# hamza1030/stereo_matching_cuda

Measured on AMD Instinct MI355X. Metric: disparity MPix/s (stereo pair -> L+R disparity + occlusion-filled map), higher is better.
Workload: dtype f32; 1 GPU; kitti 1242x375 D=192 seeded synthetic pair (seed 20150101); width=1242, height=375, disparities=192, slices_in_flight=192, walker_launches_per_call=1

## Files before the change

stereo_matching_cuda_amd/csrc/smx_agg.hip:

```cpp
#include <string.h>

#include "smx_agg.h"
#include "smx_agg_v4.h"
#include "smx_agg_v5.h"
#include "smx_launch.h"
#include "smx_wta.h"

namespace smx {

constexpr int RING_TH_COLOR_MAX = 59745, RING_TH_GRAD_MAX = 59872;

static bool ring_applies(const smx_params* p, bool use_cost) {
    return v4_supported(p) && (use_cost || (p->th_color <= RING_TH_COLOR_MAX && p->th_grad <= RING_TH_GRAD_MAX));
}

static bool v5_applies(const smx_params* p, int w, int h, int nviews, bool use_cost) {
    return v5_fix_bytes(w, h, nviews) < 0x80000000ull &&
           (use_cost ? v5_supported_cost(p) && (size_t)w * h >= 4 : v5_supported(p));
}

int agg_path_for(const smx_params* p, int w, int h, int nviews, bool use_cost, int forced, const char** why) {
    *why = nullptr;
    if (forced == 1) return 1;
    if (!ring_applies(p, use_cost)) {
// ... 69 lines not shown
static_assert(WS_SLACK >= 255 + FIT_RESERVE, "a workspace sized for n slices holds n slices");
size_t agg_workspace_bytes(int w, int h, int nslices) {
    const AggLayout L = agg_layout(w, h, v4::RMAX, 1, true, true, true, nslices);
    return L.ctrl + agg_ctrl_bytes(L.K_flags, 2 * (size_t)nslices) + WS_COMB_COPY_SLACK + WS_SLACK;
}

int agg_plan(const smx_params* p, int w, int h, int nviews, bool use_cost, bool own_q, const AggOpts& opt, size_t ws_bytes,
             size_t lost, int total, AggLayout* L) {
    const bool comb = opt.walker != 4 && v5_applies(p, w, h, nviews, use_cost);
    const bool fallback = comb && use_cost;
    const char* why = nullptr;
    if (!agg_path_for(p, w, h, nviews, use_cost, opt.walker == 5 ? 5 : 3, &why)) return fail(SMX_E_ARG, "aggregate_fused: %s", why);
    if ((size_t)h * ((size_t)w + 2 * v4::PADX) * 8 >= 0x80000000ull)
        return fail(SMX_E_ARG, "aggregate_fused: an image plane of %d x %d exceeds 2 GiB", w, h);
    const size_t avail = ws_bytes > lost ? ws_bytes - lost : 0;
    *L = agg_layout(w, h, p->radius, nviews, comb, fallback, own_q, 0);
    if (L->fg[0] > avail) return fail(SMX_E_WS, "aggregate_fused: workspace too small");
    const size_t per_sv = L->q_slice + L->hand_sv * 4 + (size_t)L->K_flags * sizeof(unsigned);
    const size_t rest = avail > L->chunk_begin ? avail - L->chunk_begin : 0;
    const size_t fit = rest > FIT_RESERVE ? (rest - FIT_RESERVE) / (per_sv * nviews) : 0;
    if (L->chunk_begin > avail || (fit < 1 && total > 0))
        return fail(SMX_E_WS, "aggregate_fused: workspace %zu B too small (need >= %zu B per view)", ws_bytes,
                    agg_workspace_bytes(w, h, 1));
    int chunk = fit > (size_t)total ? total : (int)fit;
    if (opt.max_chunk > 0 && chunk > opt.max_chunk) chunk = opt.max_chunk;
    if (chunk < 1) chunk = 1;
    *L = agg_layout(w, h, p->radius, nviews, comb, fallback, own_q, chunk);
    if (L->end > avail) return fail(SMX_E_WS, "aggregate_fused: workspace carve overflow");
    return SMX_OK;
}

int agg_read_status(const void* d_ws, unsigned* out, int nwords) {
    const char* base = (const char*)align_up((size_t)d_ws, 256);
    SMX_HIP(hipMemcpy(out, base, sizeof(unsigned) * (size_t)nwords, hipMemcpyDeviceToHost));
    return SMX_OK;
}

static v5::Args comb_args(const v4::Args& a, const AggLayout& L, char* base, bool use_cost, bool fast) {
    v5::Args b;
    memset(&b, 0, sizeof(b));
    b.fix = base + L.fg[0];
    b.fix_bytes = L.fix_end - L.fg[0];
    for (int v = 0; v < 2; ++v) {
        const int vv = v < L.nviews ? v : 0;
        b.o_fg[v] = (unsigned)(L.fg[v] - L.fg[0]);
        b.o_g1p[v] = (unsigned)(L.g1p[vv] - L.fg[0]);
        b.o_i2p[v] = (unsigned)(L.i2p[vv] - L.fg[0]);
        b.q[v] = a.v[vv].q;
        b.d0[v] = a.v[vv].d0;
        b.cost[v] = a.v[vv].cost;
    }
    b.w = a.w; b.h = a.h; b.K = L.K; b.NI = L.NI;
    b.P = v5::period(a.h, L.K);
    b.nslices = a.nslices; b.nsv = a.nsv; b.nitems = a.nitems;
    b.hand = (float*)a.hand; b.flags = a.flags; b.ticket = a.ticket; b.status = a.status;
    b.src_cost = use_cost ? 1 : 0;
    b.cost_plane = L.plane;
    b.bad = a.status + 1;
    b.cc = a.cc;
    const _Float16 hc = (_Float16)a.cc.th_color, hg = (_Float16)a.cc.th_grad;
    unsigned short uc, ug;
    memcpy(&uc, &hc, 2); memcpy(&ug, &hg, 2);
    b.th2 = (unsigned)uc | ((unsigned)ug << 16);
    b.fast = fast ? 1 : 0;
    constexpr double PRIO_MAX_Q_BYTES = 6e9;
    const double q_bytes = (double)a.nsv * (double)L.qplane * 4.0;
    b.prio = q_bytes < PRIO_MAX_Q_BYTES ? 1 : 0;
    b.qperm = L.own_q ? 1 : 0;
    b.q_plane = L.qplane;
    return b;
}

static int guidance(const AggLayout& L, char* base, const AggCall& c, v4::Guidance* out) {
    const int nviews = L.nviews, w = c.w, h = c.h;
    const smx_params* const p = c.p;
    hipStream_t st = c.st;
    v4::Guidance& g = *out;
    memset(&g, 0, sizeof(g));
    g.I[0] = c.guide[0];
    g.I[1] = nviews == 2 ? c.guide[1] : c.other[0];
    for (int i = 0; i < 2; ++i) g.FG[i] = (aggdev::fg_t*)(base + L.fg[i]);
    for (int v = 0; v < nviews; ++v) {
        g.S0[v] = (float*)(base + L.scratch[v][0]); g.S1[v] = (float*)(base + L.scratch[v][1]);
        g.G[v] = (aggdev::f2*)(base + L.guid[v]);
        g.mean_u8[v] = c.mean_u8[v];
    }
    g.zero[0] = (unsigned*)(base + L.status); g.nzero[0] = 64;
    g.zero[1] = (unsigned*)(base + L.ctrl); g.nzero[1] = (unsigned)(L.ctrl_bytes / 4);
    int rc = v4_guidance_launch(g, nviews, w, h, p->radius, p->eps, !L.comb, st);
    if (rc || !L.comb) return rc;
    aggdev::f2* g1p[2] = {nullptr, nullptr};
    unsigned* i2p[2] = {nullptr, nullptr};
    for (int v = 0; v < nviews; ++v) { g1p[v] = (aggdev::f2*)(base + L.g1p[v]); i2p[v] = (unsigned*)(base + L.i2p[v]); }
    return v5_perm_launch(nviews, g.S0, g.S1, g.G, g.mean_u8, g.FG, g1p, i2p, w, h, p->eps, st);
}

static int aggregate_fused(const AggCall& c, const AggOpts& opt, AggInfo* info) {
    const smx_params* const p = c.p;
    const int nviews = c.nviews, w = c.w, h = c.h, s_begin = c.s_begin, s_end = c.s_end;
    hipStream_t st = c.st;
    const bool use_cost = c.cost[0] != nullptr;
    const bool own_q = !c.agg[0];
    float* const* const d_nbr = c.nbr[0] ? c.nbr : nullptr;
    float* const* const d_uq = c.uq[0] ? c.uq : nullptr;
    char* const base = (char*)align_up((size_t)c.ws, 256);
    AggLayout L;
    int rc = agg_plan(p, w, h, nviews, use_cost, own_q, opt, c.ws_bytes, (size_t)(base - (char*)c.ws), s_end - s_begin, &L);
    if (rc) return rc;
    info->walker_used = L.comb ? 5 : 4;
    info->chunk = L.chunk;
    if (opt.keys_fresh && s_end <= s_begin) {
        for (int v = 0; v < nviews; ++v)
            if ((rc = launch_init_keys(c.keys[v], (int64_t)w * h, st))) return rc;
    }
    unsigned* const status = (unsigned*)(base + L.status);
    char* const ctrl = base + L.ctrl;
    v4::Guidance g;
    if ((rc = guidance(L, base, c, &g))) return rc;
    int nl = 3;
    stage_mark(ST_GUIDANCE, st);

    v4::Args a0;
    memset(&a0, 0, sizeof(a0));
    a0.w = w; a0.h = h; a0.R = p->radius; a0.K = L.K; a0.NI = L.NI;
    a0.cc = make_cost_const(p);
    for (int v = 0; v < nviews; ++v) {
        a0.v[v].FG1 = g.FG[v]; a0.v[v].FG2 = g.FG[v ^ 1];
        a0.v[v].guid = g.G[v];
    }
    a0.hand = (aggdev::f2*)(base + L.hand);
    a0.ticket = (unsigned*)ctrl; a0.status = status;
    a0.flags = (unsigned*)(ctrl + AGG_CTRL_BYTES);
    const unsigned* const fell_back = L.fallback ? status + 1 : nullptr;
    for (int s0 = s_begin; s0 < s_end; s0 += L.chunk) {
        const int cnt = (s_end - s0) < L.chunk ? (s_end - s0) : L.chunk;
        v4::Args a = a0;
        const float* q[2] = {nullptr, nullptr};
        for (int v = 0; v < nviews; ++v) {
            a.v[v].q = own_q ? (float*)(base + L.q[v]) : c.agg[v] + (size_t)(s0 - s_begin) * L.plane;
            a.v[v].d0 = c.dmin[v] + s0;
            a.v[v].cost = use_cost ? c.cost[v] + (size_t)(s0 - s_begin) * L.plane : nullptr;
            q[v] = a.v[v].q;
        }
        a.nslices = cnt; a.nsv = cnt * nviews;
        a.nitems = a.nsv * L.K;
        const size_t ctrl_bytes = agg_ctrl_bytes(L.K_flags, a.nsv);
        if (s0 != s_begin) SMX_HIP(hipMemsetAsync(ctrl, 0, ctrl_bytes, st));
        if (L.comb) {
            rc = v5_launch(comb_args(a, L, base, use_cost, opt.fast), st);
            if (!rc && L.fallback) {
                SMX_HIP(hipMemsetAsync(ctrl, 0, ctrl_bytes, st));
                v4::Args a4 = a;
                a4.K = L.K4; a4.NI = L.NI4;
                a4.nitems = a4.nsv * L.K4;
                a4.gate = fell_back;
                rc = v4_walk_launch(a4, true, opt.fast, st);
                nl += 2;
            }
        } else rc = v4_walk_launch(a, use_cost, opt.fast, st);
        if (rc) return rc;
        ++info->walker_launches;
        stage_mark(ST_WALK, st);
        const bool fresh = opt.keys_fresh && s0 == s_begin;
        const bool comb_q = L.comb && own_q;
        rc = wta_launch(comb_q ? WTA_COMB : WTA_NATURAL, nviews, q, c.keys, d_nbr, d_uq, w, h, L.qplane, cnt, s0,
                        comb_q ? fell_back : nullptr, 0, fresh, st);
        if (!rc && comb_q && L.fallback) {
// ... 112 lines not shown
```

stereo_matching_cuda_amd/csrc/smx_agg_dev.h:

```cpp
#pragma once
#include "smx_common.h"

namespace smx {
namespace aggdev {

typedef _Float16 fg_t __attribute__((ext_vector_type(2)));
typedef float f2 __attribute__((ext_vector_type(2)));
typedef float f4 __attribute__((ext_vector_type(4)));
typedef unsigned u4 __attribute__((ext_vector_type(4)));
typedef unsigned u2 __attribute__((ext_vector_type(2)));

constexpr int PADX = 4;

constexpr int RCP_N = 19 * 19 + 1;
struct RcpTable {
    float v[RCP_N];
    constexpr RcpTable() : v() {
        v[0] = 0.0f;
        for (int i = 1; i < RCP_N; ++i) v[i] = 1.0f / (float)i;
    }
};
static __constant__ RcpTable kRcp = RcpTable();

__device__ __forceinline__ float div_small_int(float x, float d, float r) {
    float q = x * r;
    float e = __builtin_fmaf(-q, d, x);
    return __builtin_fmaf(e, r, q);
}
__device__ __forceinline__ f2 div_small_int2(f2 x, float d, float r) {
    const f2 d2 = {d, d}, r2 = {r, r};
    f2 q = x * r2;
    f2 e = __builtin_elementwise_fma(-q, d2, x);
    return __builtin_elementwise_fma(e, r2, q);
}
__device__ __forceinline__ bool div_needs_exact(float x) {
    const float ax = fabsf(x);
    return !(ax >= 0x1p-100f && ax < __builtin_inff());
}

__device__ __forceinline__ f2 guid_point(const float* __restrict__ S0, const float* __restrict__ S1, int x, int y, int w, int h,
                                         int R, double eps) {
    const int ymin = max(-1, y - R - 1), ymax = min(h - 1, y + R);
    const int xmin = max(-1, x - R - 1), xmax = min(w - 1, x + R);
    const bool hx = xmin >= 0, hy = ymin >= 0;
    const size_t i11 = (size_t)ymax * w + xmax, i10 = (size_t)ymax * w + (hx ? xmin : 0);
    const size_t i01 = (size_t)(hy ? ymin : 0) * w + xmax, i00 = (size_t)(hy ? ymin : 0) * w + (hx ? xmin : 0);
    const float area = (float)((xmax - xmin) * (ymax - ymin));
    auto box = [&](const float* __restrict__ S) {
        float val = S[i11];
        if (hx) val -= S[i10];
        if (hy) val -= S[i01];
        if (hx && hy) val += S[i00];
        return 1.0f * val / area;
    };
    const float m = box(S0), sq = box(S1);
    const float m2 = m * m;
    const float var = sq - m2;
    return (f2){m, (float)(1.0f / ((double)var + eps))};
}
__device__ __forceinline__ uint8_t mean_to_u8(float m) {
    const int ci = (int)m;
    return (ci > 255) ? 255 : (uint8_t)ci;
}

__device__ __forceinline__ f2 cost_pair(fg_t q1, fg_t q2, const CostConst& cc) {
    const f2 v1 = {(float)q1.x, (float)q1.y}, v2 = {(float)q2.x, (float)q2.y};
    const f2 d = v1 - v2;
    const f2 m = {__builtin_fminf(__builtin_fabsf(d.x), cc.th_color), __builtin_fminf(__builtin_fabsf(d.y), cc.th_grad)};
    const f2 xz = (f2){cc.oma, cc.alpha} * m;
    f2 r;
    r.x = xz.x + xz.y;
    r.y = v1.x * r.x;
    return r;
}

typedef __amdgpu_buffer_rsrc_t rsrc_t;
constexpr int AUX_SC1 = 16;
constexpr int AUX_NT = 2;
__device__ __forceinline__ rsrc_t mk_rsrc(const void* p, size_t bytes) {
    return __builtin_amdgcn_make_buffer_rsrc(const_cast<void*>(p), 0,
                                             (int)(bytes > 0xFFFFFFFFull ? 0xFFFFFFFFull : bytes),
                                             0x00020000);
}
__device__ __forceinline__ f4 ld16_sc1(rsrc_t r, unsigned byteoff) {
    return __builtin_bit_cast(f4, __builtin_amdgcn_raw_buffer_load_b128(r, (int)byteoff, 0, AUX_SC1));
}
__device__ __forceinline__ void st16_sc1(rsrc_t r, unsigned byteoff, f4 v) {
    __builtin_amdgcn_raw_buffer_store_b128(__builtin_bit_cast(u4, v), r, (int)byteoff, 0, AUX_SC1);
}
__device__ __forceinline__ unsigned ldu(rsrc_t r, unsigned voff, int soff) {
    return __builtin_amdgcn_raw_buffer_load_b32(r, (int)voff, soff, 0);
}
typedef __attribute__((address_space(1))) unsigned gu32;
__device__ __forceinline__ unsigned flag_load(unsigned* p) {
    return __hip_atomic_load((gu32*)p, __ATOMIC_RELAXED, __HIP_MEMORY_SCOPE_AGENT);
}
__device__ __forceinline__ void flag_store(unsigned* p, unsigned v) {
    __hip_atomic_store((gu32*)p, v, __ATOMIC_RELAXED, __HIP_MEMORY_SCOPE_AGENT);
}
__device__ __forceinline__ void drain_vmem() { asm volatile("s_waitcnt vmcnt(0)" ::: "memory"); }
__device__ __forceinline__ void wg_barrier() {
    asm volatile("s_waitcnt lgkmcnt(0)\n\ts_barrier" ::: "memory");
}

constexpr unsigned FLAG_DONE = 0x7fffffffu;
constexpr unsigned OOB = 0x80000000u;

__device__ __forceinline__ int opaque(int x) { asm volatile("" : "+v"(x)); return x; }
typedef __attribute__((address_space(3))) const char lds_cc;
__device__ __forceinline__ unsigned lds_off(const void* p) { return (unsigned)(size_t)(lds_cc*)p; }

}
}
```

stereo_matching_cuda_amd/csrc/smx_agg_v4.hip:

```cpp
#include <stdlib.h>
#include <string.h>

#include <type_traits>

#include "smx_agg_v4.h"

namespace smx {
namespace v4 {
using namespace aggdev;

constexpr int TWMAX = OW + HWMAX;
constexpr int NCOLP = 84;
constexpr int OFF1 = 88;
constexpr int ROWF = OFF1 + NCOLP;
static_assert(NCOLP >= TWMAX && NCOLP % 4 == 0 && OFF1 % 4 == 0 && OFF1 >= NCOLP, "planar ring row");
constexpr int NT = 512;
constexpr int NWAVE = NT / 64;
constexpr int RPW = BH / NWAVE;
constexpr int RR = BH + 2 * RMAX + 2;
static_assert(RR % 4 == 0 && RR % RPW == 0 && BH % RPW == 0 && RPW % 2 == 0,
              "groups of four (column scan) and of RPW (box, cost) consecutive ring rows never wrap");

enum Src { SRC_IMG = 0, SRC_COST = 1 };

// ... 65 lines not shown
                g = 1.0f * (c2 - c1) / 2;
            }
            fg_t v;
            v.x = (_Float16)f;
            v.y = (_Float16)g;
            FGo[(size_t)(y0 + r) * wp + xp] = v;
        }
    }
    if (view >= ga.nviews) return;
    __syncthreads();
    if (tid < 2 * rows) {
        float* row = gr_lds + tid * wpad;
        float acc = -0.0f;
        f4 c[16], n[16];
        auto rd = [&](f4 (&t)[16], int x0) {
#pragma unroll
            for (int k = 0; k < 16; ++k) t[k] = *(const f4*)(row + x0 + 4 * k);
        };
        auto scan_wr = [&](f4 (&t)[16], int x0) {
#pragma unroll
            for (int k = 0; k < 16; ++k) {
                acc = t[k].x + acc; t[k].x = acc;
                acc = t[k].y + acc; t[k].y = acc;
                acc = t[k].z + acc; t[k].z = acc;
                acc = t[k].w + acc; t[k].w = acc;
            }
#pragma unroll
            for (int k = 0; k < 16; ++k) *(f4*)(row + x0 + 4 * k) = t[k];
        };
        rd(c, 0);
        for (int x0 = 0; x0 < wr; x0 += 128) {
            rd(n, x0 + 64);
            scan_wr(c, x0);
            rd(c, min(x0 + 128, wr - 64));
            scan_wr(n, x0 + 64);
        }
    }
    __syncthreads();
    for (int r = 0; r < rows; ++r) {
        if (y0 + r >= h) break;
        float* d0 = S0 + (size_t)(y0 + r) * w;
        float* d1 = S1 + (size_t)(y0 + r) * w;
        for (int x = tid; x < w; x += GR_NT) {
            d0[x] = P0[r * wpad + x];
            d1[x] = P1[r * wpad + x];
        }
    }
}

constexpr int GC_NW = 16, GC_SEG = 32;
__global__ __launch_bounds__(64 * GC_NW) void k_v4_guid_cols(GuidArgs ga, int w, int h) {
    __shared__ float s_acc[64];
    __shared__ int s_turn;
    const int lane = threadIdx.x & 63, wv = threadIdx.x >> 6;
    const int x = blockIdx.x * 64 + lane;
    const bool on = x < w;
    float* __restrict__ p = ga.S[blockIdx.z][blockIdx.y] + min(x, w - 1);
    if (threadIdx.x == 0) s_turn = 0;
    __syncthreads();
    const int nseg = (h + GC_SEG - 1) / GC_SEG;
    float v[GC_SEG];
    for (int seg = wv; seg < nseg; seg += GC_NW) {
        const int y0 = seg * GC_SEG;
#pragma unroll
        for (int t = 0; t < GC_SEG; ++t) v[t] = p[(size_t)min(y0 + t, h - 1) * w];
        while (__hip_atomic_load(&s_turn, __ATOMIC_ACQUIRE, __HIP_MEMORY_SCOPE_WORKGROUP) != seg) __builtin_amdgcn_s_sleep(1);
        float acc = seg == 0 ? -0.0f : s_acc[lane];
#pragma unroll
        for (int t = 0; t < GC_SEG; ++t) { acc = v[t] + acc; v[t] = acc; }
        s_acc[lane] = acc;
        __builtin_amdgcn_fence(__ATOMIC_RELEASE, "workgroup");
        if (lane == 0) __hip_atomic_store(&s_turn, seg + 1, __ATOMIC_RELEASE, __HIP_MEMORY_SCOPE_WORKGROUP);
        if (on) {
#pragma unroll
            for (int t = 0; t < GC_SEG; ++t)
                if (y0 + t < h) p[(size_t)(y0 + t) * w] = v[t];
        }
    }
}

__global__ void k_v4_guid_finish(GuidArgs ga, int w, int h, int R, double eps) {
    const int x = blockIdx.x * blockDim.x + threadIdx.x, y = blockIdx.y, view = blockIdx.z;
    if (x >= w) return;
    const f2 g = guid_point(ga.S[view][0], ga.S[view][1], x, y, w, h, R, eps);
    const size_t id = (size_t)y * w + x;
    ga.G[view][id] = g;
    if (ga.mean_u8[view]) ga.mean_u8[view][id] = mean_to_u8(g.x);
}

constexpr int REC_U = REC_F2 / 2;
static_assert(REC_U <= NT && HP % 2 == 0 && BH % 2 == 0, "one 16-byte hand-off unit per thread");

constexpr int NQ = (TWMAX + 3) / 4;
constexpr int QW0 = 2;
constexpr int QTH = NT - 64 * QW0;
constexpr int NQR = BH / 16;
static_assert(NQ * 4 <= NCOLP && NQ <= 4 * (NWAVE - QW0), "one wave-instruction covers 16 rows x 4 quads");

#define LDS_RD64(dst, addr, imm) asm volatile("ds_read_b64 %0, %1 offset:%2" : "=v"(dst) : "v"(addr), "i"(imm))
#define LDS_RD2(dst, addr, o0, o1) \
    asm volatile("ds_read2_b32 %0, %1 offset0:%2 offset1:%3" : "=v"(dst) : "v"(addr), "i"(o0), "i"(o1))

template <int SRC, int RT, bool FAST>
__global__ __launch_bounds__(NT, 2 * WG_PER_CU) void k_v4_walk(Args A) {
    __shared__ __attribute__((aligned(16))) float ring1[RR * ROWF];
    __shared__ __attribute__((aligned(16))) float ring2[RR * ROWF];
    __shared__ __attribute__((aligned(16))) f2 cout[2][BH];
    __shared__ __attribute__((aligned(16))) f2 cin_fast[FAST ? 2 : 1][FAST ? BH : 1];
    __shared__ float rcp_s[HWMAX * HWMAX + 1];
    __shared__ int s_item, s_next;
    __shared__ unsigned s_seen;

    const int tid = threadIdx.x, lane = tid & 63;
    const int wave = __builtin_amdgcn_readfirstlane(tid >> 6);
    const int w = A.w, h = A.h, K = A.K, NI = A.NI, nsv = A.nsv;
    const int R = RT >= 0 ? RT : A.R;
    const int HW = 2 * R + 1, TW = OW + HW;
    const CostConst cc = A.cc;
    const f2 ident = {-0.0f, -0.0f};
    if (tid <= HWMAX * HWMAX) rcp_s[tid] = kRcp.v[tid];

    const int qt = tid - 64 * QW0;
    constexpr int NHALO_U = BH * HP / 2;
    static_assert(NHALO_U + BH <= QTH, "one hand-off unit per thread of waves QW0..");
    const bool hu_halo = qt >= 0 && qt < NHALO_U;
    const bool hu_carry = qt >= NHALO_U && qt < NHALO_U + BH;
    auto hu_rc = [&](int& r, int& c) {
        const int u = max(opaque(qt), 0);
        r = u / (HP / 2);
        c = (u - r * (HP / 2)) * 2;
    };
    auto hu_off = [&]() {
        const int u = opaque(qt);
        return u < NHALO_U ? (unsigned)(2 * BH * 8 + u * 16) : (unsigned)((u - NHALO_U) * 16);
    };
    auto srow_of = [&]() { return opaque(lane) & 15; };
    auto scomp_of = [&]() { return (opaque(lane) >> 4) & 1; };
    auto sstage_of = [&]() { return opaque(lane) >> 5; };
    constexpr int NRSW = 1;
    const bool q_on = wave >= QW0 && 4 * (wave - QW0) + (lane >> 4) < NQ;
    auto quad_rc = [&](int e, int& r, int& c) {
        const int l = opaque(lane);
        r = 16 * e + (l & 15);
        c = (4 * (wave - QW0) + (l >> 4)) * 4;
    };

    if (A.gate && flag_load(const_cast<unsigned*>(A.gate)) == 0u) return;
    if (tid == 0) s_item = (int)__hip_atomic_fetch_add((gu32*)A.ticket, 1u, __ATOMIC_RELAXED, __HIP_MEMORY_SCOPE_AGENT);
    for (;;) {
        wg_barrier();
        const int item = s_item;
        if (item >= A.nitems) break;
        const int k = item / nsv;
        const int sv = item - k * nsv;
        const int view = sv / A.nslices;
        const int slice = sv - view * A.nslices;
        const View& V = A.v[view];
        const int xs = k * OW;
        const int cs1 = xs - R - 1;
        const int cs2 = xs - HW;
        const bool pred = k > 0, succ = k + 1 < K;
        const int d = V.d0 + slice;
        unsigned* const myflag = A.flags + (size_t)sv * K + k;
        const size_t recs = (size_t)NI * REC_F2;
        const rsrc_t r_in = mk_rsrc(A.hand + ((size_t)((k - 1) & 1) * nsv + sv) * recs, recs * 8);
        const rsrc_t r_out = mk_rsrc(A.hand + ((size_t)(k & 1) * nsv + sv) * recs, recs * 8);

// ... 655 lines not shown
```

stereo_matching_cuda_amd/csrc/smx_agg_v5.hip:

```cpp
#include <stdlib.h>
#include <string.h>

#include <type_traits>

#include "smx_agg_dev.h"
#include "smx_agg_v5.h"
#include "smx_v5_diag.h"

namespace smx {
namespace v5 {
using namespace aggdev;

constexpr int SWU = HW * L;
constexpr int SW = (SWU + 3) / 4 * 4;
static_assert(OWS == HW * (L - 1) && SWU == OWS + HW && CPW * L <= 64 && CPW * NS1 >= HW, "strip geometry");
constexpr int RD = 20;
static_assert(RD % BH == 0 && RD >= HW + 1, "ring");
static_assert(L == 9, "the shipped form: seven combs of nine lanes per comb wave");
constexpr int NX = 2;
constexpr int NWAVE = 2 * NS1 + NX, NT = 64 * NWAVE;
constexpr int WPE = 4;
constexpr int NT1 = 3, NT2 = 2;
enum Role { ROLE_S1 = 0, ROLE_S2 = 1, ROLE_SCAN = 2, ROLE_COST = 3 };
constexpr int P1 = (SW + 63) / 64 * 64;
// ... 748 lines not shown
                        if (nxt < A.nitems) {
                            const int kn = nxt / nsv, svn = nxt - kn * nsv;
                            if (kn > 0) pn = flag_load(A.flags + (size_t)svn * K + kn - 1);
                        }
                        s_peekn = pn;
                    }
                }
                if (A.prio) __builtin_amdgcn_s_setprio(PRIO_COST);
                if (own && slf + 2 < NI) eval_band_p(slf + 2, G1[2]);
                __builtin_amdgcn_s_setprio(0);
            } else if constexpr (ROLE == ROLE_S1) {
                if (own) slot_s1(PARc, slf);
            } else {
                const int sl = sl2;
                if (own && sl >= 1 && sl <= q_last) {
                    slot_s2(PARc, sl);
                } else if (lane == 0) {
                    __hip_atomic_fetch_add(&s_x1, 1u, __ATOMIC_RELAXED, __HIP_MEMORY_SCOPE_WORKGROUP);
                }
            }
            have_pref = f_pred && (seen == FLAG_DONE || seen >= (unsigned)(slf + 3));
            if (f_pred && !have_pref && slf + 2 < NI) {
                if (tid == 0) spin_pred((unsigned)(slf + 3));
                wg_barrier();
                seen = s_seen;
                if constexpr (ROLE == ROLE_S1) {
                    const int hq = hu_idx();
                    const f4 late = ld16_sc1(r_hand, (unsigned)(o_in + min(slf + 2, NI - 1) * REC_U * 16) + (hq >= 0 && hq < REC_U ? (unsigned)hq * 16u : 0u));
                    cin1 = GC[1]; tile2 = G2[0];
                    hand_in(slf >= 0, late);
                }
            } else if constexpr (ROLE == ROLE_S1) {
                V5_MARK("s1handin begin");
                if (own && pred && slf + 2 < NI) { cin1 = GC[1]; tile2 = G2[0]; hand_in(slf >= 0, hreg); }
                V5_MARK("s1handin end");
            }
            if constexpr (ROLE == ROLE_S1) {
                g1_load(slf >= 0 ? 5 * slf + 6 : slf + 2, PARc);
                if (own && slf == 0 && succ) drain_vmem();
            }
            V5_STAMP(5);
            if (ending && slf == 1) return true;
            { float* const t = G1[0]; G1[0] = G1[1]; G1[1] = G1[2]; G1[2] = t; }
            { float* const t = G2[0]; G2[0] = G2[1]; G2[1] = t; }
            { float (*const t)[2] = GC[0]; GC[0] = GC[1]; GC[1] = t; }
            ++g;
            ++sl2;
            return false;
        };
        for (;;) {
            bool done = false;
            for (slf = -2; slf < 2 && !done; slf += 2) {
                done = iter(std::integral_constant<int, 0>{});
                if (!done) { ++slf; done = iter(std::integral_constant<int, 1>{}); --slf; }
            }
            if (done) break;
            for (slf = 2; slf <= P - 3; slf += 2) {
                (void)iter(std::integral_constant<int, 0>{});
                ++slf;
                (void)iter(std::integral_constant<int, 1>{});
                --slf;
            }
            ++nf;
        }
        if constexpr (ROLE == ROLE_COST) { if (own) cost_verdict(); }
        };
        if (wave < NS1) item_body(std::integral_constant<int, ROLE_S1>{});
        else if (wave < 2 * NS1) item_body(std::integral_constant<int, ROLE_S2>{});
        else if (wave == 2 * NS1) item_body(std::integral_constant<int, ROLE_SCAN>{});
        else item_body(std::integral_constant<int, ROLE_COST>{});
    }
}

struct PermArgs {
    const float* S0[2];
    const float* S1[2];
    f2* G[2];
    uint8_t* mean_u8[2];
    double eps;
    const fg_t* FG[2];
    f2* g1p[2];
    unsigned* i2p[2];
};
__global__ __launch_bounds__(CLP) void k_v5_perm(PermArgs pa, int w, int h, int K, int NI) {
    const int cl = threadIdx.x, cw = cl >> 6, ln = cl & 63;
    const int rho = ln / L < CPW ? CPW * cw + ln / L : HW, il = ln % L;
    const int kb = blockIdx.x / (BH / 2), j = blockIdx.x - kb * (BH / 2);
    const int k = kb / NI, ib = kb - k * NI, v = blockIdx.y;
    const int x1 = OWS * k - R - 1 + HW * il + rho;
    const int xq = x1 - R;
    const bool on1 = rho < HW && x1 >= 0 && x1 < w, on2 = rho < HW && xq >= 0 && xq < w;
    {
        const int ya = min(max(BH * ib - R + 2 * j, 0), h - 1), yb = min(max(BH * ib - R + 2 * j + 1, 0), h - 1);
        f4 g = {0.0f, 0.0f, 0.0f, 0.0f};
        if (on1) {
            const f2 a = guid_point(pa.S0[v], pa.S1[v], x1, ya, w, h, R, pa.eps);
            const f2 b = yb == ya ? a : guid_point(pa.S0[v], pa.S1[v], x1, yb, w, h, R, pa.eps);
            g = (f4){a.x, a.y, b.x, b.y};
            pa.G[v][(size_t)ya * w + x1] = a;
            pa.G[v][(size_t)yb * w + x1] = b;
            if (pa.mean_u8[v]) {
                pa.mean_u8[v][(size_t)ya * w + x1] = mean_to_u8(a.x);
                pa.mean_u8[v][(size_t)yb * w + x1] = mean_to_u8(b.x);
            }
        }
        ((f4*)pa.g1p[v])[((size_t)k * (5 * NI) + 5 * ib + j) * CLP + cl] = g;
    }
    {
        const int yp = min(max((BH * (ib - 1) - 2 * R) / 2 + j, 0), (h - 1) / 2), y = 2 * yp;
        fg_t p2 = {(_Float16)0.0f, (_Float16)0.0f};
        if (on2) {
            p2.x = pa.FG[v][(size_t)y * (w + 2 * PADX) + PADX + xq].x;
            if (y + 1 < h) p2.y = pa.FG[v][(size_t)(y + 1) * (w + 2 * PADX) + PADX + xq].x;
        }
        const unsigned pr = __builtin_bit_cast(unsigned, p2);
        unsigned* const i2a = pa.i2p[v];
        unsigned* const i2b = pa.i2p[v] + (size_t)K * NI * CLP * 4;
        const size_t e = ((size_t)k * NI + ib) * CLP + cl;
        if (j < 4) i2a[4 * e + j] = pr; else i2b[e] = pr;
    }
}

}

int v5_perm_launch(int nviews, const float* const* S0, const float* const* S1, aggdev::f2* const* G, uint8_t* const* mean_u8,
                   const aggdev::fg_t* const* FG, aggdev::f2* const* g1p, unsigned* const* i2p, int w, int h, double eps,
                   hipStream_t st) {
    v5::PermArgs pa;
    memset(&pa, 0, sizeof(pa));
    for (int v = 0; v < nviews; ++v) {
        pa.S0[v] = S0[v]; pa.S1[v] = S1[v]; pa.G[v] = G[v]; pa.mean_u8[v] = mean_u8[v];
        pa.FG[v] = FG[v]; pa.g1p[v] = g1p[v]; pa.i2p[v] = i2p[v];
    }
    pa.eps = eps;
    const int K = v5::strips(w), NI = v5::bands(h);
    hipLaunchKernelGGL(v5::k_v5_perm, dim3((unsigned)(K * NI * (v5::BH / 2)), (unsigned)nviews), dim3(v5::CLP), 0, st, pa, w, h, K, NI);
    SMX_HIP(hipGetLastError());
    return SMX_OK;
}

void v5_slots(int h, int K, int* bands, int* q_last, int* period) { *bands = v5::bands(h); *q_last = (h + 37) / 10; *period = v5::period(h, K); }

bool v5_supported(const smx_params* p) {
    if (p->radius != v5::R) return false;
    if (!(p->eps >= 1.0) || !(p->eps < 1e30)) return false;
    const CostConst c = make_cost_const(p);
    if (!(c.alpha >= 0.0f && c.alpha <= 1.0f && c.th_color >= 0.0f && c.th_color < 1e6f && c.th_grad >= 0.0f && c.th_grad < 1e6f))
        return false;
    const float m1 = c.th_color < 1.0f ? c.th_color : 1.0f, m2 = c.th_grad < 0.5f ? c.th_grad : 0.5f;
    const float t1 = c.oma * m1, t2 = c.alpha * m2;
    auto ok = [](float t) { return t == 0.0f || t >= 0x1p-60f; };
    if (!(ok(t1) && ok(t2))) return false;
    if (!((float)(_Float16)c.th_color == c.th_color && (float)(_Float16)c.th_grad == c.th_grad && c.th_color <= 59744.0f &&
          c.th_grad <= 59872.0f))
        return false;
    return true;
}

bool v5_supported_cost(const smx_params* p) { return p->radius == v5::R && p->eps >= 1.0 && p->eps < 1e30; }

int v5_launch(const v5::Args& a, hipStream_t st) {
    int dev = 0, ncu = 256;
    SMX_HIP(hipGetDevice(&dev));
    SMX_HIP(hipDeviceGetAttribute(&ncu, hipDeviceAttributeMultiprocessorCount, dev));
    const int slots = v5::WG_PER_CU * ncu;
    const int grid = a.nitems < slots ? a.nitems : slots;
    if (a.fast && a.qperm) hipLaunchKernelGGL((v5::k_v5_walk<1, 1>), dim3((unsigned)grid), dim3(v5::NT), 0, st, a);
    else if (a.fast) hipLaunchKernelGGL((v5::k_v5_walk<1, 0>), dim3((unsigned)grid), dim3(v5::NT), 0, st, a);
    else if (a.qperm) hipLaunchKernelGGL((v5::k_v5_walk<0, 1>), dim3((unsigned)grid), dim3(v5::NT), 0, st, a);
    else hipLaunchKernelGGL((v5::k_v5_walk<0, 0>), dim3((unsigned)grid), dim3(v5::NT), 0, st, a);
    SMX_HIP(hipGetLastError());
    return SMX_OK;
}

extern "C" __attribute__((visibility("default"))) int smx_debug_v5_occupancy(int* blocks_per_cu, int* vgprs, int* lds_bytes) {
    int nb = 0;
    SMX_HIP(hipOccupancyMaxActiveBlocksPerMultiprocessor(&nb, (const void*)v5::k_v5_walk<0, 1>, v5::NT, 0));
    hipFuncAttributes fa;
    SMX_HIP(hipFuncGetAttributes(&fa, (const void*)v5::k_v5_walk<0, 1>));
    if (blocks_per_cu) *blocks_per_cu = nb;
    if (vgprs) *vgprs = fa.numRegs;
    if (lds_bytes) *lds_bytes = (int)fa.sharedSizeBytes;
    return SMX_OK;
}

}
```

stereo_matching_cuda_amd/csrc/smx_kernels.hip:

```cpp
#include "smx_common.h"
#include "smx_wta.h"

namespace smx {

__global__ void k_gray(const uint8_t* __restrict__ rgb, int64_t n, int ch,
                       uint8_t* __restrict__ gray, double rw, double gw, double bw) {
    int64_t k = (int64_t)blockIdx.x * blockDim.x + threadIdx.x;
    if (k >= n) return;
    const uint8_t* px = rgb + (int64_t)ch * k;
    double val = rw * px[0] + gw * px[1] + bw * px[2];
    gray[k] = (uint8_t)val;
}

__device__ __forceinline__ float xgrad(const uint8_t* __restrict__ row, int x, int w) {
    int c1, c2;
    if (x - 1 >= 0 && x + 1 < w) { c1 = row[x + 1]; c2 = row[x - 1]; }
    else if (x + 1 >= w)         { c1 = row[x];     c2 = row[x - 1]; }
    else                         { c1 = row[x + 1]; c2 = row[x];     }
    return 1.0f * (float)(c2 - c1) / 2;
}

__device__ __forceinline__ float cost_cell(const uint8_t* __restrict__ r1,
                                           const uint8_t* __restrict__ r2, int x, int d, int w1,
                                           int w2, float g1, const CostConst& cc) {
// ... 262 lines not shown
    if (key != KEY_IDENTITY) {
        float q;
        uint32_t s;
        unpack_key(key, &q, &s);
        if (1.0f * b >= 1.0f * q) {
            d = (float)((k < n ? dminl : dminr) + (int)s);
            b = q;
        }
    }
    best[k] = b;
    dmap[k] = d;
    if (k < n) occlusion[k] = d;
}

__global__ void k_detect_occlusion(float* dL, const float* __restrict__ dR, int dOcclusion, int w,
                                   int h, int d_lr) {
    int x = blockIdx.x * blockDim.x + threadIdx.x;
    int y = blockIdx.y;
    if (x >= w) return;
    int64_t id = (int64_t)y * w + x;
    int d = (int)dL[id];
    if (x + d < 0 || x + d >= w || fabsf((float)d + dR[id + d]) > (float)d_lr)
        dL[id] = (float)dOcclusion;
}

__global__ __launch_bounds__(64) void k_fill_occlusion(const float* in, float* disp, int w, int h, float vMin) {
    extern __shared__ float sbuf[];
    float* sLeft = sbuf;
    float* sVal = sbuf + w;
    const int lane = threadIdx.x;
    const float* row = in + (int64_t)blockIdx.x * w;
    float* out = disp + (int64_t)blockIdx.x * w;
    for (int x = lane; x < w; x += 64) sVal[x] = row[x];
    __syncthreads();
    float carry = vMin;
    for (int c0 = 0; c0 < w; c0 += 64) {
        int x = c0 + lane;
        float v = x < w ? sVal[x] : 0.0f;
        bool valid = x < w && v >= vMin;
        unsigned long long mask = __ballot(valid);
        unsigned long long lower = mask & ((2ull << lane) - 1ull);
        int src = lower ? 63 - __clzll((long long)lower) : lane;
        float pick = __shfl(v, src);
        if (x < w) sLeft[x] = lower ? pick : carry;
        int last = mask ? 63 - __clzll((long long)mask) : 0;
        float nv = __shfl(v, last);
        if (mask) carry = nv;
    }
    carry = vMin;
    for (int c0 = ((w - 1) / 64) * 64; c0 >= 0; c0 -= 64) {
        int x = c0 + lane;
        float v = x < w ? sVal[x] : 0.0f;
        bool valid = x < w && v >= vMin;
        unsigned long long mask = __ballot(valid);
        unsigned long long upper = mask & (~0ull << lane);
        int src = upper ? __ffsll((long long)upper) - 1 : lane;
        float pick = __shfl(v, src);
        float right = upper ? pick : carry;
        if (x < w) {
            int dX = (int)v;
            if (!((float)dX >= vMin)) {
                float l = sLeft[x];
                out[x] = l > right ? l : right;
            } else if (in != disp) {
                out[x] = v;
            }
        }
        int first = mask ? __ffsll((long long)mask) - 1 : 0;
        float nv = __shfl(v, first);
        if (mask) carry = nv;
    }
}

constexpr int FP_NT = 256;
constexpr int FP_MAXW = 8192;
__global__ __launch_bounds__(FP_NT) void k_finish_pair_row(const int64_t* __restrict__ keys, int w, int h, int dminl,
                                                            int dminr, int dOcclusion, int d_lr, float vMin,
                                                            float* __restrict__ best, float* __restrict__ dmap,
                                                            float* __restrict__ occlusion, float* __restrict__ filled) {
    extern __shared__ float sbuf[];
    float* sVal = sbuf;
    float* sR = sbuf + w;
    float* sLeft = sbuf + 2 * w;
    const int tid = threadIdx.x, y = blockIdx.x;
    const int64_t n = (int64_t)w * h, r0 = (int64_t)y * w;
    auto decode = [&](int64_t key, int dmin, float& b, float& d) {
        b = __builtin_bit_cast(float, 0x7F7F7F7Fu);
        d = 0.0f;
        if (key != KEY_IDENTITY) {
            float q;
            uint32_t s;
            unpack_key(key, &q, &s);
            if (1.0f * b >= 1.0f * q) {
                d = (float)(dmin + (int)s);
                b = q;
            }
        }
    };
    for (int x0 = 0; x0 < w; x0 += 4 * FP_NT) {
        int64_t kl[4], kr[4];
#pragma unroll
        for (int t = 0; t < 4; ++t) {
            const int x = min(x0 + t * FP_NT + tid, w - 1);
            kl[t] = keys[r0 + x];
            kr[t] = keys[n + r0 + x];
        }
#pragma unroll
        for (int t = 0; t < 4; ++t) {
            const int x = x0 + t * FP_NT + tid;
            if (x < w) {
                float b, d;
                decode(kl[t], dminl, b, d);
                best[r0 + x] = b;
                dmap[r0 + x] = d;
                sVal[x] = d;
                decode(kr[t], dminr, b, d);
                best[n + r0 + x] = b;
                dmap[n + r0 + x] = d;
                sR[x] = d;
            }
        }
    }
    __syncthreads();
    for (int x = tid; x < w; x += FP_NT) {
        float v = sVal[x];
        const int d = (int)v;
        if (x + d < 0 || x + d >= w || fabsf((float)d + sR[x + d]) > (float)d_lr) v = (float)dOcclusion;
        sVal[x] = v;
        occlusion[r0 + x] = v;
    }
    __syncthreads();
    if (tid >= 64) return;
    const int lane = tid;
    float* out = filled + r0;
    float carry = vMin;
    for (int c0 = 0; c0 < w; c0 += 64) {
        int x = c0 + lane;
        float v = x < w ? sVal[x] : 0.0f;
        bool valid = x < w && v >= vMin;
        unsigned long long mask = __ballot(valid);
        unsigned long long lower = mask & ((2ull << lane) - 1ull);
        int src = lower ? 63 - __clzll((long long)lower) : lane;
        float pick = __shfl(v, src);
        if (x < w) sLeft[x] = lower ? pick : carry;
        int last = mask ? 63 - __clzll((long long)mask) : 0;
        float nv = __shfl(v, last);
        if (mask) carry = nv;
    }
    carry = vMin;
    for (int c0 = ((w - 1) / 64) * 64; c0 >= 0; c0 -= 64) {
        int x = c0 + lane;
        float v = x < w ? sVal[x] : 0.0f;
        bool valid = x < w && v >= vMin;
        unsigned long long mask = __ballot(valid);
        unsigned long long upper = mask & (~0ull << lane);
        int src = upper ? __ffsll((long long)upper) - 1 : lane;
        float pick = __shfl(v, src);
        float right = upper ? pick : carry;
        if (x < w) {
            int dX = (int)v;
            if (!((float)dX >= vMin)) {
                float l = sLeft[x];
                out[x] = l > right ? l : right;
            } else {
                out[x] = v;
            }
        }
        int first = mask ? __ffsll((long long)mask) - 1 : 0;
        float nv = __shfl(v, first);
        if (mask) carry = nv;
    }
}

__global__ void k_filter(const uint8_t* __restrict__ I, uint8_t* __restrict__ mean,
                         float* __restrict__ var, int w, int h, int R) {
    const int x = blockIdx.x * blockDim.x + threadIdx.x;
    const int y = blockIdx.y;
    if (x >= w) return;
    float s1 = 0.0f, s2 = 0.0f;
    for (int ix = -R; ix <= R; ++ix) {
        const int xx = x + ix;
        for (int iy = -R; iy <= R; ++iy) {
            const int yy = y + iy;
            float v = 0.0f, v2 = 0.0f;
            if (xx >= 0 && xx < w && yy >= 0 && yy < h) {
                const int c = (int)I[(int64_t)yy * w + xx];
                v = (float)c;
                v2 = (float)(c * c);
            }
            s1 += v;
            s2 += v2;
        }
    }
    const int area = (2 * R + 1) * (2 * R + 1);
    const int m = (int)(s1 / area);
    const int m2 = (int)(s2 / area);
    const uint8_t mu = (uint8_t)m;
    const int64_t id = (int64_t)y * w + x;
    mean[id] = mu;
    const float mm = (float)((int)mu * (int)mu);
    var[id] = (float)m2 - mm;
}

}

namespace smx {

static inline unsigned cdiv(int64_t a, int64_t b) { return (unsigned)((a + b - 1) / b); }

int launch_gray(const smx_params* p, const uint8_t* rgb, int64_t n, int ch, uint8_t* gray,
                hipStream_t st) {
    hipLaunchKernelGGL(k_gray, dim3(cdiv(n, 256)), dim3(256), 0, st, rgb, n, ch, gray, p->r_w,
                       p->g_w, p->b_w);
    SMX_HIP(hipGetLastError());
    return SMX_OK;
}

int launch_cost(const smx_params* p, const uint8_t* i1, const uint8_t* i2, float* cost, int w,
                int h, int d0, int count, hipStream_t st) {
    if (count <= 0) return SMX_OK;
    CostConst cc = make_cost_const(p);
    dim3 grid(cdiv(w, 256), h, cdiv(count, COST_ZPER));
    hipLaunchKernelGGL(k_cost, grid, dim3(256), 0, st, i1, i2, cost, w, h, d0, count, cc);
    SMX_HIP(hipGetLastError());
    return SMX_OK;
}

int launch_integral(int mode, const float* in0, const float* in1, float* out0, float* out1, int w,
                    int h, int nplanes, hipStream_t st) {
    if (nplanes <= 0) return SMX_OK;
    const int bands = (h + 63) / 64;
    dim3 grid((unsigned)(bands * (int64_t)nplanes));
    if (mode == 0)
        hipLaunchKernelGGL(k_rowscan<0>, grid, dim3(64), 0, st, in0, in1, out0, out1, w, h, nplanes);
    else if (mode == 1)
        hipLaunchKernelGGL(k_rowscan<1>, grid, dim3(64), 0, st, in0, in1, out0, out1, w, h, nplanes);
    else
        hipLaunchKernelGGL(k_rowscan<2>, grid, dim3(64), 0, st, in0, in1, out0, out1, w, h, nplanes);
    SMX_HIP(hipGetLastError());
    dim3 cgrid(cdiv((int64_t)nplanes * w, 256), mode == 0 ? 1 : 2);
    hipLaunchKernelGGL(k_colscan, cgrid, dim3(256), 0, st, out0, out1, w, h, nplanes);
    SMX_HIP(hipGetLastError());
    return SMX_OK;
}

int launch_guid_finish(const smx_params* p, const float* S_im, const float* S_sq, float* mean_im,
                       float* cinv, uint8_t* mean_u8, int w, int h, hipStream_t st) {
    dim3 grid(cdiv(w, 256), h);
    hipLaunchKernelGGL(k_guid_finish, grid, dim3(256), 0, st, S_im, S_sq, mean_im, cinv, mean_u8, w,
                       h, p->radius, p->eps);
    SMX_HIP(hipGetLastError());
    return SMX_OK;
}
// ... 4 lines not shown
    return SMX_OK;
}

int launch_ab(const smx_params* p, const float* Sp, const float* SIp, const float* mean_im,
              const float* cinv, float* A, float* B, int w, int h, int nplanes, hipStream_t st) {
    if (nplanes <= 0) return SMX_OK;
    dim3 grid(cdiv(w, 256), h, nplanes);
    hipLaunchKernelGGL(k_ab, grid, dim3(256), 0, st, Sp, SIp, mean_im, cinv, A, B, w, h, p->radius);
    SMX_HIP(hipGetLastError());
    return SMX_OK;
}

int launch_q_wta(const smx_params* p, const float* Sa, const float* Sb, const float* im,
                 int64_t* keys, float* nbr, float* uq, float* agg, int w, int h, int count, int slice0, hipStream_t st) {
    if (count <= 0) return SMX_OK;
    dim3 grid(cdiv(w, 256), h);
    auto go = [&](auto kernel) {
        hipLaunchKernelGGL(kernel, grid, dim3(256), 0, st, Sa, Sb, im, keys, nbr, uq, agg, w, h, count, slice0, p->radius);
    };
    if (nbr && uq) go(k_q_wta<true, true>);
    else if (uq) go(k_q_wta<false, true>);
    else if (nbr) go(k_q_wta<true, false>);
    else go(k_q_wta<false, false>);
    SMX_HIP(hipGetLastError());
    return SMX_OK;
}

int launch_init_keys(int64_t* keys, int64_t n, hipStream_t st) {
    hipLaunchKernelGGL(k_init_keys, dim3(cdiv(n, 256)), dim3(256), 0, st, keys, n);
    SMX_HIP(hipGetLastError());
    return SMX_OK;
}

int launch_init_wta(float* best, float* dmap, int64_t n, hipStream_t st) {
    hipLaunchKernelGGL(k_init_wta, dim3(cdiv(n, 256)), dim3(256), 0, st, best, dmap, n);
    SMX_HIP(hipGetLastError());
    return SMX_OK;
}

int launch_apply_keys(const int64_t* keys, int64_t n, int dmin, float* best, float* dmap,
                      hipStream_t st) {
    hipLaunchKernelGGL(k_apply_keys, dim3(cdiv(n, 256)), dim3(256), 0, st, keys, n, dmin, best,
                       dmap);
    SMX_HIP(hipGetLastError());
    return SMX_OK;
}

int launch_detect_occlusion(const smx_params* p, float* dL, const float* dR, int dOcc, int w, int h,
                            hipStream_t st) {
    dim3 grid(cdiv(w, 256), h);
    hipLaunchKernelGGL(k_detect_occlusion, grid, dim3(256), 0, st, dL, dR, dOcc, w, h, p->d_lr);
    SMX_HIP(hipGetLastError());
    return SMX_OK;
}

int launch_filter(const smx_params* p, const uint8_t* I, uint8_t* mean, float* var, int w, int h,
                  hipStream_t st) {
    hipLaunchKernelGGL(k_filter, dim3(cdiv(w, 256), h), dim3(256), 0, st, I, mean, var, w, h, p->radius);
    SMX_HIP(hipGetLastError());
    return SMX_OK;
}

int launch_fill_occlusion(const float* src, float* disp, int w, int h, float vMin, hipStream_t st) {
    size_t lds = (size_t)w * 2 * sizeof(float);
    if (lds > 128 * 1024) return fail(SMX_E_ARG, "fill_occlusion: width %d exceeds LDS row buffer", w);
    static LdsLimitOnce lim;
    if (lds > 64 * 1024) SMX_HIP(lim.ensure((const void*)k_fill_occlusion, 128 * 1024));
    hipLaunchKernelGGL(k_fill_occlusion, dim3(h), dim3(64), lds, st, src, disp, w, h, vMin);
    SMX_HIP(hipGetLastError());
    return SMX_OK;
}

int launch_finish_keys(const int64_t* keys, int64_t n, int dminl, int dminr, float* best, float* dmap,
                       float* occlusion, hipStream_t st) {
    hipLaunchKernelGGL(k_finish_keys, dim3(cdiv(2 * n, 256)), dim3(256), 0, st, keys, n, dminl, dminr, best, dmap,
                       occlusion);
    SMX_HIP(hipGetLastError());
    return SMX_OK;
}

bool finish_pair_row_supported(int w) { return w <= FP_MAXW; }
int launch_finish_pair_row(const smx_params* p, const int64_t* keys, int w, int h, int dminl, int dminr, int dOcc,
                           float vMin, float* best, float* dmap, float* occlusion, float* filled, hipStream_t st) {
    const size_t lds = (size_t)w * 3 * sizeof(float);
    static LdsLimitOnce lim;
    if (lds > 64 * 1024) SMX_HIP(lim.ensure((const void*)k_finish_pair_row, (int)((size_t)FP_MAXW * 3 * sizeof(float))));
    hipLaunchKernelGGL(k_finish_pair_row, dim3(h), dim3(FP_NT), lds, st, keys, w, h, dminl, dminr, dOcc, p->d_lr, vMin,
                       best, dmap, occlusion, filled);
    SMX_HIP(hipGetLastError());
    return SMX_OK;
}

}
```

Before: 591.1 MPix/s.

## Stage guidance box-filter taps in LDS and parallelize occlusion fill scans

The permutation kernel now cooperatively loads the four integral-image rows needed for each pair of output rows into shared memory and evaluates the box filter from LDS, instead of issuing scattered global loads per thread. The guidance G and mean outputs are written through a shared-memory staging buffer so stores are coalesced, and G is skipped entirely when the combined path makes it unnecessary. In the finish-row kernel, the left and right hole-fill scans run concurrently on two wavefronts, and the final selection is done by all threads. The cost is extra LDS, additional barriers, and a larger per-block LDS footprint.

```diff
diff --git a/stereo_matching_cuda_amd/csrc/smx_agg.hip b/stereo_matching_cuda_amd/csrc/smx_agg.hip
--- a/stereo_matching_cuda_amd/csrc/smx_agg.hip
+++ b/stereo_matching_cuda_amd/csrc/smx_agg.hip
@@ -175,7 +175,7 @@
     for (int i = 0; i < 2; ++i) g.FG[i] = (aggdev::fg_t*)(base + L.fg[i]);
     for (int v = 0; v < nviews; ++v) {
         g.S0[v] = (float*)(base + L.scratch[v][0]); g.S1[v] = (float*)(base + L.scratch[v][1]);
-        g.G[v] = (aggdev::f2*)(base + L.guid[v]);
+        g.G[v] = L.comb && !L.fallback ? nullptr : (aggdev::f2*)(base + L.guid[v]);
         g.mean_u8[v] = c.mean_u8[v];
     }
     g.zero[0] = (unsigned*)(base + L.status); g.nzero[0] = 64;
diff --git a/stereo_matching_cuda_amd/csrc/smx_agg_dev.h b/stereo_matching_cuda_amd/csrc/smx_agg_dev.h
--- a/stereo_matching_cuda_amd/csrc/smx_agg_dev.h
+++ b/stereo_matching_cuda_amd/csrc/smx_agg_dev.h
@@ -38,27 +38,42 @@
     return !(ax >= 0x1p-100f && ax < __builtin_inff());
 }
 
-__device__ __forceinline__ f2 guid_point(const float* __restrict__ S0, const float* __restrict__ S1, int x, int y, int w, int h,
-                                         int R, double eps) {
+struct GuidTapGlobal {
+    const float* __restrict__ S0;
+    const float* __restrict__ S1;
+    int w;
+    __host__ __device__ __forceinline__ float operator()(int plane, bool , int yy, int xx) const {
+        return (plane ? S1 : S0)[(size_t)yy * w + xx];
+    }
+};
+template <int NC>
+struct GuidTapStaged {
+    const float (*rows)[2][NC];
+    int c0;
+    __host__ __device__ __forceinline__ float operator()(int plane, bool lower, int , int xx) const {
+        return rows[lower ? 1 : 0][plane][xx - c0];
+    }
+};
+template <class Tap>
+__host__ __device__ __forceinline__ f2 guid_point(const Tap& tap, int x, int y, int w, int h, int R, double eps) {
     const int ymin = max(-1, y - R - 1), ymax = min(h - 1, y + R);
     const int xmin = max(-1, x - R - 1), xmax = min(w - 1, x + R);
     const bool hx = xmin >= 0, hy = ymin >= 0;
-    const size_t i11 = (size_t)ymax * w + xmax, i10 = (size_t)ymax * w + (hx ? xmin : 0);
-    const size_t i01 = (size_t)(hy ? ymin : 0) * w + xmax, i00 = (size_t)(hy ? ymin : 0) * w + (hx ? xmin : 0);
+    const int xl = hx ? xmin : 0, yt = hy ? ymin : 0;
     const float area = (float)((xmax - xmin) * (ymax - ymin));
-    auto box = [&](const float* __restrict__ S) {
-        float val = S[i11];
-        if (hx) val -= S[i10];
-        if (hy) val -= S[i01];
-        if (hx && hy) val += S[i00];
+    auto box = [&](int plane) {
+        float val = tap(plane, true, ymax, xmax);
+        if (hx) val -= tap(plane, true, ymax, xl);
+        if (hy) val -= tap(plane, false, yt, xmax);
+        if (hx && hy) val += tap(plane, false, yt, xl);
         return 1.0f * val / area;
     };
-    const float m = box(S0), sq = box(S1);
+    const float m = box(0), sq = box(1);
     const float m2 = m * m;
     const float var = sq - m2;
     return (f2){m, (float)(1.0f / ((double)var + eps))};
 }
-__device__ __forceinline__ uint8_t mean_to_u8(float m) {
+__host__ __device__ __forceinline__ uint8_t mean_to_u8(float m) {
     const int ci = (int)m;
     return (ci > 255) ? 255 : (uint8_t)ci;
 }
diff --git a/stereo_matching_cuda_amd/csrc/smx_agg_v4.hip b/stereo_matching_cuda_amd/csrc/smx_agg_v4.hip
--- a/stereo_matching_cuda_amd/csrc/smx_agg_v4.hip
+++ b/stereo_matching_cuda_amd/csrc/smx_agg_v4.hip
@@ -171,7 +171,7 @@
 __global__ void k_v4_guid_finish(GuidArgs ga, int w, int h, int R, double eps) {
     const int x = blockIdx.x * blockDim.x + threadIdx.x, y = blockIdx.y, view = blockIdx.z;
     if (x >= w) return;
-    const f2 g = guid_point(ga.S[view][0], ga.S[view][1], x, y, w, h, R, eps);
+    const f2 g = guid_point(GuidTapGlobal{ga.S[view][0], ga.S[view][1], w}, x, y, w, h, R, eps);
     const size_t id = (size_t)y * w + x;
     ga.G[view][id] = g;
     if (ga.mean_u8[view]) ga.mean_u8[view][id] = mean_to_u8(g.x);
diff --git a/stereo_matching_cuda_amd/csrc/smx_agg_v5.hip b/stereo_matching_cuda_amd/csrc/smx_agg_v5.hip
--- a/stereo_matching_cuda_amd/csrc/smx_agg_v5.hip
+++ b/stereo_matching_cuda_amd/csrc/smx_agg_v5.hip
@@ -854,7 +854,12 @@
     f2* g1p[2];
     unsigned* i2p[2];
 };
+constexpr int PTW = OWS + 2 * HW;
+constexpr int PNC = OWS + HW;
+static_assert(PTW <= CLP && PNC <= CLP, "one staged column per thread");
 __global__ __launch_bounds__(CLP) void k_v5_perm(PermArgs pa, int w, int h, int K, int NI) {
+    __shared__ float s_tap[4][2][CLP];
+    __shared__ f2 s_out[2][CLP];
     const int cl = threadIdx.x, cw = cl >> 6, ln = cl & 63;
     const int rho = ln / L < CPW ? CPW * cw + ln / L : HW, il = ln % L;
     const int kb = blockIdx.x / (BH / 2), j = blockIdx.x - kb * (BH / 2);
@@ -864,19 +869,48 @@
     const bool on1 = rho < HW && x1 >= 0 && x1 < w, on2 = rho < HW && xq >= 0 && xq < w;
     {
         const int ya = min(max(BH * ib - R + 2 * j, 0), h - 1), yb = min(max(BH * ib - R + 2 * j + 1, 0), h - 1);
+        const int c0 = OWS * k - 2 * R - 2;
+        {
+            const int yr[4] = {ya - R - 1, min(ya + R, h - 1), yb - R - 1, min(yb + R, h - 1)};
+            const int xx = c0 + cl;
+            const bool onx = cl < PTW && xx >= 0 && xx < w;
+            float t[4][2];
+#pragma unroll
+            for (int s = 0; s < 4; ++s) {
+                const bool ld = onx && yr[s] >= 0 && (s < 2 || yb != ya);
+                t[s][0] = ld ? pa.S0[v][(size_t)yr[s] * w + xx] : 0.0f;
+                t[s][1] = ld ? pa.S1[v][(size_t)yr[s] * w + xx] : 0.0f;
+            }
+#pragma unroll
+            for (int s = 0; s < 4; ++s) { s_tap[s][0][cl] = t[s][0]; s_tap[s][1][cl] = t[s][1]; }
+        }
+        __syncthreads();
         f4 g = {0.0f, 0.0f, 0.0f, 0.0f};
         if (on1) {
-            const f2 a = guid_point(pa.S0[v], pa.S1[v], x1, ya, w, h, R, pa.eps);
-            const f2 b = yb == ya ? a : guid_point(pa.S0[v], pa.S1[v], x1, yb, w, h, R, pa.eps);
+            const f2 a = guid_point(GuidTapStaged<CLP>{&s_tap[0], c0}, x1, ya, w, h, R, pa.eps);
+            const f2 b = yb == ya ? a : guid_point(GuidTapStaged<CLP>{&s_tap[2], c0}, x1, yb, w, h, R, pa.eps);
             g = (f4){a.x, a.y, b.x, b.y};
-            pa.G[v][(size_t)ya * w + x1] = a;
-            pa.G[v][(size_t)yb * w + x1] = b;
-            if (pa.mean_u8[v]) {
-                pa.mean_u8[v][(size_t)ya * w + x1] = mean_to_u8(a.x);
-                pa.mean_u8[v][(size_t)yb * w + x1] = mean_to_u8(b.x);
-            }
         }
         ((f4*)pa.g1p[v])[((size_t)k * (5 * NI) + 5 * ib + j) * CLP + cl] = g;
+        if (pa.G[v] || pa.mean_u8[v]) {
+            if (on1) {
+                s_out[0][x1 - (c0 + R + 1)] = (f2){g.x, g.y};
+                s_out[1][x1 - (c0 + R + 1)] = (f2){g.z, g.w};
+            }
+            __syncthreads();
+            const int xo = c0 + R + 1 + cl;
+            if (cl < PNC && xo >= 0 && xo < w) {
+                const f2 a = s_out[0][cl], b = s_out[1][cl];
+                if (pa.G[v]) {
+                    pa.G[v][(size_t)ya * w + xo] = a;
+                    pa.G[v][(size_t)yb * w + xo] = b;
+                }
+                if (pa.mean_u8[v]) {
+                    pa.mean_u8[v][(size_t)ya * w + xo] = mean_to_u8(a.x);
+                    pa.mean_u8[v][(size_t)yb * w + xo] = mean_to_u8(b.x);
+                }
+            }
+        }
     }
     {
         const int yp = min(max((BH * (ib - 1) - 2 * R) / 2 + j, 0), (h - 1) / 2), y = 2 * yp;
diff --git a/stereo_matching_cuda_amd/csrc/smx_kernels.hip b/stereo_matching_cuda_amd/csrc/smx_kernels.hip
--- a/stereo_matching_cuda_amd/csrc/smx_kernels.hip
+++ b/stereo_matching_cuda_amd/csrc/smx_kernels.hip
@@ -368,6 +368,7 @@
     float* sVal = sbuf;
     float* sR = sbuf + w;
     float* sLeft = sbuf + 2 * w;
+    float* sRight = sbuf + 3 * w;
     const int tid = threadIdx.x, y = blockIdx.x;
     const int64_t n = (int64_t)w * h, r0 = (int64_t)y * w;
     auto decode = [&](int64_t key, int dmin, float& b, float& d) {
@@ -416,45 +417,49 @@
         occlusion[r0 + x] = v;
     }
     __syncthreads();
-    if (tid >= 64) return;
-    const int lane = tid;
+    const int lane = tid & 63;
+    if (tid < 64) {
+        float carry = vMin;
+        for (int c0 = 0; c0 < w; c0 += 64) {
+            int x = c0 + lane;
+            float v = x < w ? sVal[x] : 0.0f;
+            bool valid = x < w && v >= vMin;
+            unsigned long long mask = __ballot(valid);
+            unsigned long long lower = mask & ((2ull << lane) - 1ull);
+            int src = lower ? 63 - __clzll((long long)lower) : lane;
+            float pick = __shfl(v, src);
+            if (x < w) sLeft[x] = lower ? pick : carry;
+            int last = mask ? 63 - __clzll((long long)mask) : 0;
+            float nv = __shfl(v, last);
+            if (mask) carry = nv;
+        }
+    } else if (tid < 128) {
+        float carry = vMin;
+        for (int c0 = ((w - 1) / 64) * 64; c0 >= 0; c0 -= 64) {
+            int x = c0 + lane;
+            float v = x < w ? sVal[x] : 0.0f;
+            bool valid = x < w && v >= vMin;
+            unsigned long long mask = __ballot(valid);
+            unsigned long long upper = mask & (~0ull << lane);
+            int src = upper ? __ffsll((long long)upper) - 1 : lane;
+            float pick = __shfl(v, src);
+            if (x < w) sRight[x] = upper ? pick : carry;
+            int first = mask ? __ffsll((long long)mask) - 1 : 0;
+            float nv = __shfl(v, first);
+            if (mask) carry = nv;
+        }
+    }
+    __syncthreads();
     float* out = filled + r0;
-    float carry = vMin;
-    for (int c0 = 0; c0 < w; c0 += 64) {
-        int x = c0 + lane;
-        float v = x < w ? sVal[x] : 0.0f;
-        bool valid = x < w && v >= vMin;
-        unsigned long long mask = __ballot(valid);
-        unsigned long long lower = mask & ((2ull << lane) - 1ull);
-        int src = lower ? 63 - __clzll((long long)lower) : lane;
-        float pick = __shfl(v, src);
-        if (x < w) sLeft[x] = lower ? pick : carry;
-        int last = mask ? 63 - __clzll((long long)mask) : 0;
-        float nv = __shfl(v, last);
-        if (mask) carry = nv;
-    }
-    carry = vMin;
-    for (int c0 = ((w - 1) / 64) * 64; c0 >= 0; c0 -= 64) {
-        int x = c0 + lane;
-        float v = x < w ? sVal[x] : 0.0f;
-        bool valid = x < w && v >= vMin;
-        unsigned long long mask = __ballot(valid);
-        unsigned long long upper = mask & (~0ull << lane);
-        int src = upper ? __ffsll((long long)upper) - 1 : lane;
-        float pick = __shfl(v, src);
-        float right = upper ? pick : carry;
-        if (x < w) {
-            int dX = (int)v;
-            if (!((float)dX >= vMin)) {
-                float l = sLeft[x];
-                out[x] = l > right ? l : right;
-            } else {
-                out[x] = v;
-            }
-        }
-        int first = mask ? __ffsll((long long)mask) - 1 : 0;
-        float nv = __shfl(v, first);
-        if (mask) carry = nv;
+    for (int x = tid; x < w; x += FP_NT) {
+        const float v = sVal[x];
+        const int dX = (int)v;
+        if (!((float)dX >= vMin)) {
+            const float l = sLeft[x], right = sRight[x];
+            out[x] = l > right ? l : right;
+        } else {
+            out[x] = v;
+        }
     }
 }
 
@@ -625,9 +630,9 @@
 bool finish_pair_row_supported(int w) { return w <= FP_MAXW; }
 int launch_finish_pair_row(const smx_params* p, const int64_t* keys, int w, int h, int dminl, int dminr, int dOcc,
                            float vMin, float* best, float* dmap, float* occlusion, float* filled, hipStream_t st) {
-    const size_t lds = (size_t)w * 3 * sizeof(float);
+    const size_t lds = (size_t)w * 4 * sizeof(float);
     static LdsLimitOnce lim;
-    if (lds > 64 * 1024) SMX_HIP(lim.ensure((const void*)k_finish_pair_row, (int)((size_t)FP_MAXW * 3 * sizeof(float))));
+    if (lds > 64 * 1024) SMX_HIP(lim.ensure((const void*)k_finish_pair_row, (int)((size_t)FP_MAXW * 4 * sizeof(float))));
     hipLaunchKernelGGL(k_finish_pair_row, dim3(h), dim3(FP_NT), lds, st, keys, w, h, dminl, dminr, dOcc, p->d_lr, vMin,
                        best, dmap, occlusion, filled);
     SMX_HIP(hipGetLastError());
```

Measured after the change: 596.1 MPix/s (median of 6 runs). About the same (+0.8%).
